# simeoncarstens/binf

Hardware: AMD Instinct MI355X
Metric: chain*leapfrog-steps/sec, 1024-d Gaussian (higher is better)
Workload: dtype f64

## Files before the change

binf_amd/csrc/hmc_gauss.hip:

```cpp
#include "hmc_gauss_kernel.hpp"

namespace binf {

template <int TMAX, bool REGULAR, int LW, bool UDT = false, int HC = -1, bool FS = false>
static hipError_t launch_n_trl(const GaussNArgs &a, bool unit, bool fma, dim3 grid,
                               hipStream_t st)
{
    constexpr int BS = (LW == 3) ? 512 : 256;
    constexpr int R = GAUSS_RNG_HBM;
    constexpr bool FU = FS && gauss_fastsum_built(TMAX, HC, true);
    constexpr bool FN = FS && gauss_fastsum_built(TMAX, HC, false);
    if (unit) {
        if (fma) hmc_gauss_persist_kernel<TMAX, REGULAR, true, true, LW, R, UDT, HC, FU><<<grid, BS, 0, st>>>(a);
        else     hmc_gauss_persist_kernel<TMAX, REGULAR, true, false, LW, R, UDT, HC, FU><<<grid, BS, 0, st>>>(a);
    } else {
        if (fma) hmc_gauss_persist_kernel<TMAX, REGULAR, false, true, LW, R, UDT, HC, FN><<<grid, BS, 0, st>>>(a);
        else     hmc_gauss_persist_kernel<TMAX, REGULAR, false, false, LW, R, UDT, HC, FN><<<grid, BS, 0, st>>>(a);
    }
    return hipGetLastError();
}

static bool gauss_uniform_dt(const GaussNArgs &a)
{
    return a.dt_chain == nullptr && a.n_adapt == 0;
}

template <int TMAX, int HC>
static hipError_t launch_n_th(const GaussNArgs &a, bool unit, bool fma, dim3 grid,
                              hipStream_t st)
{
    if constexpr (HC == 3) {
        if (a.e_before == nullptr && a.e_after == nullptr) {
            if constexpr (TMAX == 16) {
                if (unit && gauss_uniform_dt(a) && gauss_onesum_domain(a)) {
                    constexpr int R = GAUSS_RNG_HBM;
                    if (fma) hmc_gauss_persist_kernel<16, true, true, true, 0, R, true, 3, true, true><<<grid, 256, 0, st>>>(a);
                    else     hmc_gauss_persist_kernel<16, true, true, false, 0, R, true, 3, true, true><<<grid, 256, 0, st>>>(a);
                    return hipGetLastError();
                }
            }
            if (gauss_uniform_dt(a))
                return launch_n_trl<TMAX, true, 0, true, HC, true>(a, unit, fma, grid, st);
            return launch_n_trl<TMAX, true, 0, false, HC, true>(a, unit, fma, grid, st);
        }
    }
    if (gauss_uniform_dt(a))
        return launch_n_trl<TMAX, true, 0, true, HC>(a, unit, fma, grid, st);
    return launch_n_trl<TMAX, true, 0, false, HC>(a, unit, fma, grid, st);
}

template <int TMAX>
static hipError_t launch_n_t(const GaussNArgs &a, bool regular, bool unit, bool fma,
                             dim3 grid, hipStream_t st)
{
    if (!regular)
        return launch_n_trl<TMAX, false, 0>(a, unit, fma, grid, st);
    if (a.H == 0) return launch_n_th<TMAX, 0>(a, unit, fma, grid, st);
    if constexpr (TMAX >= 12) {
        if (a.H == 1) return launch_n_th<TMAX, 1>(a, unit, fma, grid, st);
        if (a.H == 2) return launch_n_th<TMAX, 2>(a, unit, fma, grid, st);
        if (a.H == 3) return launch_n_th<TMAX, 3>(a, unit, fma, grid, st);
    }
    return hipErrorNotSupported;
}

template <int LW>
static hipError_t launch_n_wide(const GaussNArgs &a, bool regular, bool unit, bool fma,
                                dim3 grid, hipStream_t st)
{
    return regular ? launch_n_trl<16, true, LW>(a, unit, fma, grid, st)
                   : launch_n_trl<16, false, LW>(a, unit, fma, grid, st);
}

}

using namespace binf;

extern "C" int32_t binf_hmc_sample_n_gauss_f64(
    const double *q0, const double *p0, const double *u, double *q_out,
    double *samples, uint8_t *accepted, int64_t *n_accepted, double *e_before,
    double *e_after, double timestep, double *dt_chain, int64_t C, int64_t D,
    int32_t nsteps, int32_t n, int32_t thin, double k, double x0,
    int32_t n_adapt, double uprate, double downrate, int32_t mode, void *stream)
{
    if (C < 0 || D < 1 || nsteps < 1 || n < 1 || thin < 1 || n_adapt < 0)
        return fail(BINF_E_ARG, "hmc_sample_gauss: need C>=0, D>=1, nsteps>=1, n>=1, thin>=1, n_adapt>=0");
    if (mode != BINF_MODE_EXACT && mode != BINF_MODE_FMA)
        return fail(BINF_E_ARG, "hmc_sample_gauss: unknown mode %d", mode);
    if (C == 0) return 0;
    if (!q0 || !p0 || !u || !q_out)
        return fail(BINF_E_ARG, "hmc_sample_gauss: null buffer");
    if (n_adapt > 0 && !dt_chain)
        return fail(BINF_E_ARG, "hmc_sample_gauss: adaption needs dt_chain");
    if (D > 8192)
        return fail(BINF_E_UNSUPPORTED, "hmc_sample_gauss: D=%lld > 8192 not covered by the fused kernel", (long long)D);
    const GaussPlan plan = gauss_plan(C, D);
    const int32_t H = plan.H;
    if (H > 6)
        return fail(BINF_E_UNSUPPORTED, "hmc_sample_gauss: pairwise tree height %d > 6 for D=%lld", H, (long long)D);
    const int LW = plan.LW;
    const int64_t bytes = C * D * (int64_t)sizeof(double);
    const char *qo = (const char *)q_out, *qi = (const char *)q0, *pi = (const char *)p0;
    if ((qo != qi && qo < qi + bytes && qi < qo + bytes) ||
        (qo < pi + bytes * n && pi < qo + bytes))
        return fail(BINF_E_ALIAS, "hmc_sample_gauss: q_out overlaps q0/p0 (only q_out == q0 is allowed)");

    const int tneed = plan.tneed;
    const bool regular = plan.regular;
    GaussNArgs a;
    a.q0 = q0; a.p0 = p0; a.u = u; a.q_out = q_out; a.samples = samples;
    a.accepted = accepted; a.n_accepted = n_accepted; a.e_before = e_before;
    a.e_after = e_after; a.dt_chain = dt_chain; a.timestep = timestep; a.k = k;
    a.x0 = x0; a.uprate = uprate; a.downrate = downrate; a.C = C;
    a.D = (int32_t)D; a.nsteps = nsteps; a.H = H; a.n = n; a.thin = thin;
    a.n_adapt = n_adapt < n ? n_adapt : n;
    a.rng_seed = 0; a.rng_offset = 0; a.chain_offset = 0; a.p_dump = nullptr; a.u_dump = nullptr;
    gauss_derived_args(a);

    const int64_t blocks = plan.blocks;
    if (blocks > 0x7fffffffLL)
        return fail(BINF_E_UNSUPPORTED, "hmc_sample_gauss: too many chains");
    dim3 grid((unsigned)blocks);
    hipStream_t st = (hipStream_t)stream;
    const bool unit = (k == 1.0 && x0 == 0.0);
    const bool fma = (mode == BINF_MODE_FMA);
    hipError_t e;
    const int split = (LW == 0) ? gauss_split_factor(C, H, regular, tneed) : 1;
    if (split > 1)        e = launch_gauss_split(a, tneed, split, unit, fma, st);
    else if (LW == 1)     e = launch_n_wide<1>(a, regular && tneed == 16, unit, fma, grid, st);
    else if (LW == 2)     e = launch_n_wide<2>(a, regular && tneed == 16, unit, fma, grid, st);
    else if (LW == 3)     e = launch_n_wide<3>(a, regular && tneed == 16, unit, fma, grid, st);
    else if (tneed <= 1)  e = launch_n_t<1>(a, regular && tneed == 1, unit, fma, grid, st);
    else if (tneed <= 2)  e = launch_n_t<2>(a, regular && tneed == 2, unit, fma, grid, st);
    else if (tneed <= 4)  e = launch_n_t<4>(a, regular && tneed == 4, unit, fma, grid, st);
    else if (tneed <= 8)  e = launch_n_t<8>(a, regular && tneed == 8, unit, fma, grid, st);
    else if (tneed <= 12) e = launch_n_t<12>(a, regular && tneed == 12, unit, fma, grid, st);
    else                  e = launch_n_t<16>(a, regular && tneed == 16, unit, fma, grid, st);
    if (e != hipSuccess) return hip_fail(e, "hmc_gauss_persist_kernel launch");
    return 0;
}

extern "C" int32_t binf_hmc_gauss_waves_per_chain(int64_t C, int64_t D)
{
    if (C < 1 || D < 1 || D > 8192) return 0;
    const GaussPlan p = gauss_plan(C, D);
    if (p.H > 6) return 0;
    if (p.LW > 0) return 1 << p.LW;
    return gauss_split_factor(C, p.H, p.regular, p.tneed);
}

extern "C" int32_t binf_hmc_sample_gauss_f64(
    const double *q0, const double *p0, const double *u, double *q_out,
    uint8_t *accepted, int64_t *n_accepted, double *e_before, double *e_after,
    double timestep, double *dt_chain, int64_t C, int64_t D, int32_t nsteps,
    double k, double x0, int32_t adapt, double uprate, double downrate,
    int32_t mode, void *stream)
{
    if (C > 0 && D >= 1 && nsteps >= 1 && q0 && p0 && u && q_out && !accepted)
        return fail(BINF_E_ARG, "hmc_sample_gauss: null buffer");
    return binf_hmc_sample_n_gauss_f64(q0, p0, u, q_out, nullptr, accepted,
                                       n_accepted, e_before, e_after, timestep,
                                       dt_chain, C, D, nsteps, 1, 1, k, x0,
                                       adapt ? 1 : 0, uprate, downrate, mode,
                                       stream);
}
```

binf_amd/csrc/hmc_gauss_kernel.hpp:

```cpp
#pragma once
#include "gauss_common.hpp"
#include "xoshiro.hpp"

namespace binf {

enum { GAUSS_RNG_HBM = 0, GAUSS_RNG_FUSED = 1, GAUSS_RNG_DUMP = 2 };

constexpr int gauss_wpb(int LW, int RNG) { return (LW == 3 || RNG != GAUSS_RNG_HBM) ? 8 : 4; }

constexpr int GAUSS_STEP_UNROLL = 4;
constexpr int gauss_step_unroll(int TMAX, bool REGULAR, bool UNIT, bool FMA, int LW, int RNG)
{
    if (!REGULAR || LW != 0 || !UNIT) return 1;
    if ((TMAX == 12 && !FMA) || (TMAX == 4 && RNG == GAUSS_RNG_FUSED)) return 1;
    return GAUSS_STEP_UNROLL;
}

constexpr int GAUSS_PRIO_WINDOW = 4;
constexpr bool gauss_wave_priority(int LW, int RNG, int HC)
{
    return LW == 0 && RNG == GAUSS_RNG_HBM && HC == 3;
}

__device__ __forceinline__ void gauss_set_priority(int prio)
{
    switch (prio & 3) {
    case 0: __builtin_amdgcn_s_setprio(0); break;
    case 1: __builtin_amdgcn_s_setprio(1); break;
    case 2: __builtin_amdgcn_s_setprio(2); break;
    default: __builtin_amdgcn_s_setprio(3); break;
    }
}

constexpr int GAUSS_REDO_GS = 2;
template <int TMAX, int GS, bool UNIT, bool FMA>
__device__ inline bool gauss_exact_accept(const GaussNArgs &a, const double *qs, const double (*qs_lds)[64],
                                          int lane, const double *pc, double dt, double hdt, double c_lp,
                                          double u)
{
    LaneSum s0 = {0.0, 0.0}, spb = {0.0, 0.0}, sqa = {0.0, 0.0}, spa = {0.0, 0.0};
#pragma unroll 1
    for (int g = 0; g < TMAX / GS; ++g) {
        double qq[GS], pp[GS];
#pragma unroll
        for (int i = 0; i < GS; ++i) {
            const int t = g * GS + i;
            qq[i] = qs_lds ? qs_lds[t][lane] : qs[8 * t];
            pp[i] = pc[8 * t];
        }
#pragma unroll
        for (int i = 0; i < GS; ++i) {
            const int t = g * GS + i;
            const double d = UNIT ? qq[i] : qq[i] - a.x0;
            lane_sum_add<true>(s0, d * d, t, TMAX);
            lane_sum_add<true>(spb, pp[i] * pp[i], t, TMAX);
        }
#pragma unroll
        for (int i = 0; i < GS; ++i)
            pp[i] = kick<FMA>(pp[i], hdt, gauss_grad<UNIT>(qq[i], a.k, a.x0));
#pragma unroll 1
        for (int l = 0; l < a.nsteps - 1; ++l) {
#pragma unroll
            for (int i = 0; i < GS; ++i) {
                qq[i] = drift<FMA>(qq[i], pp[i], dt);
                pp[i] = kick<FMA>(pp[i], dt, gauss_grad<UNIT>(qq[i], a.k, a.x0));
            }
        }
#pragma unroll
        for (int i = 0; i < GS; ++i) {
            const int t = g * GS + i;
            qq[i] = drift<FMA>(qq[i], pp[i], dt);
            pp[i] = kick<FMA>(pp[i], hdt, gauss_grad<UNIT>(qq[i], a.k, a.x0));
            const double d = UNIT ? qq[i] : qq[i] - a.x0;
            lane_sum_add<true>(sqa, d * d, t, TMAX);
            lane_sum_add<true>(spa, pp[i] * pp[i], t, TMAX);
        }
    }
    const double r = chain_sums_shared(sqa.r, spa.r, spb.r, s0.r, true);
    const double Eb = -(c_lp * lane_value_f64<12>(r)) + 0.5 * lane_value_f64<8>(r);
    const double Ea = -(c_lp * lane_value_f64<0>(r)) + 0.5 * lane_value_f64<4>(r);
    return metropolis_accept<true>(u, -(Ea - Eb));
}

constexpr bool gauss_fastsum_built(int TMAX, int HC, bool UNIT) { return HC == 3 && (TMAX == 16 || !UNIT); }

template <int TMAX, bool REGULAR, bool UNIT, bool FMA, int LW, int RNG = GAUSS_RNG_HBM, bool UDT = false,
          int HC = -1, bool FASTSUM = false, bool ONESUM = false>
__global__ void __launch_bounds__(64 * gauss_wpb(LW, RNG))
hmc_gauss_persist_kernel(const GaussNArgs a)
{
    static_assert(HC < 0 || (REGULAR && LW == 0), "compile-time tree height: regular one-wave chains only");
    constexpr bool FIXED = HC >= 0;
    constexpr int HF = FIXED ? HC : 0;
    constexpr bool SHARED = HC == 3;
    static_assert(!FASTSUM || (SHARED && RNG == GAUSS_RNG_HBM), "fused sums: the shared-tree kernels, draws from HBM");
    static_assert(!ONESUM || (FASTSUM && UNIT && UDT), "two sums: the unit Gaussian, one step size for the batch");
    constexpr bool EARLY = FIXED && UNIT && !SHARED;
    constexpr int WPB = gauss_wpb(LW, RNG);
    constexpr int WPC = 1 << LW;
    __shared__ double xch[WPB];
    __shared__ double ubc[WPB];
    constexpr int GS = (TMAX % 8 == 0) ? 8 : ((TMAX % 4 == 0) ? 4 : TMAX);
    constexpr int NG = TMAX / GS;
    constexpr int USTEP = gauss_step_unroll(TMAX, REGULAR, UNIT, FMA, LW, RNG);
    constexpr bool PRIO = gauss_wave_priority(LW, RNG, HC);
    __shared__ double stash[RNG == GAUSS_RNG_DUMP ? 1 : WPB][RNG == GAUSS_RNG_DUMP ? 1 : TMAX][64];
    __shared__ double zx[RNG == GAUSS_RNG_HBM ? 1 : XZIG_C + 1];
    if (RNG != GAUSS_RNG_HBM) {
        xzig_load_table(zx, threadIdx.x, WPB * 64);
        __syncthreads();
    }

    const int lane = threadIdx.x & 63;
    const int wib = threadIdx.x >> 6;
    const int64_t wave = (int64_t)blockIdx.x * WPB + wib;
    const int H = FIXED ? HC : a.H;
    const int lg = (LW > 0) ? 6 : 3 + H;
    const int slot = lane & ((1 << lg) - 1);
    const int j = slot & 7;
    const int wchain = wib & (WPC - 1);
    const int grp = (LW > 0) ? ((wchain << 3) | (lane >> 3)) : (slot >> 3);
    const bool writer = (LW > 0) ? (wchain == 0 && lane == 0) : (slot == 0);

    int off, n, leafdepth, canonical;
    if (REGULAR) {
        n = 8 * TMAX;
        off = grp * n;
        leafdepth = H;
        canonical = 1;
    } else {
        const Leaf L = pairwise_leaf(a.D, H, grp);
        off = L.off;
        n = L.len;
        leafdepth = L.depth;
        canonical = L.canonical;
    }
    const int T = (n >= 8) ? (n >> 3) : 0;
    const int rem = (n >= 8) ? (n & 7) : n;

    const int64_t raw = (LW > 0) ? (int64_t)blockIdx.x * (WPB / WPC) + (wib >> LW)
                                 : (wave << (6 - lg)) + (lane >> lg);
    const bool cvalid = raw < a.C;
    const int64_t chain = cvalid ? raw : a.C - 1;
    const int64_t CD = a.C * (int64_t)a.D;
    const int64_t base = chain * (int64_t)a.D + off + j;

    double dt = (UDT || !a.dt_chain) ? a.timestep : a.dt_chain[chain];
    double uu = 0.0;
    if (RNG == GAUSS_RNG_HBM) uu = a.u[chain];
    Xo128 gen = {0u, 0u, 0u, 0u};
    uint64_t gen_stream = 0;
    if (RNG != GAUSS_RNG_HBM) {
        const int cgrp = grp & ~((1 << (H - leafdepth)) - 1);
        gen_stream = (uint64_t)(chain + a.chain_offset) * (uint64_t)(8 << H) + (uint64_t)(cgrp * 8 + j);
    }
    __builtin_amdgcn_sched_barrier(0);

    double q[TMAX], pa[GS], pb[GS];
#pragma unroll
    for (int t = 0; t < GS; ++t) {
        const bool m = REGULAR || (8 * t + j < n);
        q[t] = (m && RNG != GAUSS_RNG_DUMP) ? a.q0[base + 8 * t] : 0.0;
    }
    if (RNG == GAUSS_RNG_HBM) {
#pragma unroll
        for (int i = 0; i < GS; ++i) {
            const bool m = REGULAR || (8 * i + j < n);
            pa[i] = m ? a.p0[base + 8 * i] : 0.0;
        }
    }
#pragma unroll
    for (int t = GS; t < TMAX; ++t) {
        const bool m = REGULAR || (8 * t + j < n);
        q[t] = (m && RNG != GAUSS_RNG_DUMP) ? a.q0[base + 8 * t] : 0.0;
    }

    const double c_lp = SHARED ? a.c_lp : -0.5 * a.k;
    LaneSum s0 = {0.0, 0.0};
    double Sq_state = 0.0;
    int64_t nacc = 0;

    const bool stash_lds = !(REGULAR && ((a.samples && a.thin == 1) || a.n == 1));
    double *rec = a.samples;
    const double *prev = a.q0;
    int rec_wait = a.thin;

    for (int s = 0; s < a.n; ++s) {
        if (PRIO) {
            const int left = (a.n - 1 - s) / GAUSS_PRIO_WINDOW;
            gauss_set_priority(left < 3 ? left : 3);
        }
        const double hdt = (UDT && SHARED) ? a.half_timestep : 0.5 * dt;
        if (RNG != GAUSS_RNG_HBM) gen = xo_seed(gen_stream, a.rng_seed, a.rng_offset + (uint64_t)s);
        if (RNG != GAUSS_RNG_DUMP && stash_lds) {
#pragma unroll
            for (int t = 0; t < TMAX; ++t) stash[wib][t][lane] = q[t];
        }

        const bool more = s + 1 < a.n;
        const double *pc = a.p0 + (int64_t)s * CD + base;
        const double *pn = more ? pc + CD : pc;
        double un = 0.0;
        if (RNG == GAUSS_RNG_HBM) un = a.u[(int64_t)(more ? s + 1 : s) * a.C + chain];

        LaneSum spb = {0.0, 0.0}, sqa = {0.0, 0.0}, spa = {0.0, 0.0};
        double Spb = 0.0;
#pragma unroll
        for (int g = 0; g < NG; ++g) {
            double(&cur)[GS] = (RNG == GAUSS_RNG_HBM && (g & 1)) ? pb : pa;
            double(&nxt)[GS] = (RNG == GAUSS_RNG_HBM && (g & 1)) ? pa : pb;
            if (RNG != GAUSS_RNG_HBM) {
                unsigned want = 0;
#pragma unroll
                for (int i = 0; i < GS; ++i)
                    if (REGULAR || (8 * (g * GS + i) + j < n)) want |= 1u << i;
                xzig_normals<GS>(cur, want, gen, zx);
                if (RNG == GAUSS_RNG_DUMP) {
                    if (cvalid && canonical) {
                        double *go = a.p_dump + (int64_t)s * CD + base;
#pragma unroll
                        for (int i = 0; i < GS; ++i)
                            if (want & (1u << i)) go[8 * (g * GS + i)] = cur[i];
                    }
                    continue;
                }
            } else if (g + 1 < NG) {
#pragma unroll
                for (int i = 0; i < GS; ++i) {
                    const int t = (g + 1) * GS + i;
                    const bool m = REGULAR || (8 * t + j < n);
                    nxt[i] = m ? pc[8 * t] : 0.0;
                }
            } else {
#pragma unroll
                for (int i = 0; i < GS; ++i) {
                    const bool m = REGULAR || (8 * i + j < n);
                    nxt[i] = m ? pn[8 * i] : 0.0;
                }
            }
            (void)nxt;
#pragma unroll
            for (int i = 0; i < GS; ++i)
                asm volatile("" : "+v"(cur[i]), "+v"(q[g * GS + i]));
            if (s == 0) {
#pragma unroll
                for (int i = 0; i < GS; ++i) {
                    const int t = g * GS + i;
                    const double d = UNIT ? q[t] : q[t] - a.x0;
                    if (FASTSUM) lane_sum_fused(s0, d, t);
                    else lane_sum_add<REGULAR>(s0, d * d, t, T);
                }
                if (FIXED && !SHARED && g == NG - 1) {
                    double v[1] = {s0.r};
                    chain_sum_finish_fixed<HF, 1>(v, lane);
                    Sq_state = v[0];
                }
            }
#pragma unroll
            for (int i = 0; i < GS; ++i) {
                if (FASTSUM) lane_sum_fused(spb, cur[i], g * GS + i);
                else lane_sum_add<REGULAR>(spb, cur[i] * cur[i], g * GS + i, T);
            }
            __builtin_amdgcn_sched_barrier(0);
            if (EARLY && g == NG - 1) {
                double v[1] = {spb.r};
                chain_sum_finish_fixed<HF, 1>(v, lane);
                Spb = v[0];
            }
#pragma unroll
            for (int i = 0; i < GS; ++i) {
                const int t = g * GS + i;
                cur[i] = kick<FMA>(cur[i], hdt, gauss_grad<UNIT>(q[t], a.k, a.x0));
            }
            if (EARLY && g == NG - 1) asm volatile("" : "+v"(Spb));
            if (USTEP == 1) {
                for (int l = 0; l < a.nsteps - 1; ++l) {
#pragma unroll
                    for (int i = 0; i < GS; ++i) {
                        const int t = g * GS + i;
                        q[t] = drift<FMA>(q[t], cur[i], dt);
                        cur[i] = kick<FMA>(cur[i], dt, gauss_grad<UNIT>(q[t], a.k, a.x0));
                    }
                }
            } else {
                const auto step = [&]() {
#pragma unroll
                    for (int i = 0; i < GS; ++i) {
                        const int t = g * GS + i;
                        q[t] = drift<FMA>(q[t], cur[i], dt);
                        cur[i] = kick<FMA>(cur[i], dt, gauss_grad<UNIT>(q[t], a.k, a.x0));
                    }
                };
                static_assert((USTEP & (USTEP - 1)) == 0, "the remainder below goes by the bits of its count");
                const int nl = a.nsteps > 1 ? a.nsteps - 1 : 0;
#pragma unroll 1
                for (int m = nl / USTEP; m > 0; --m) {
#pragma unroll
                    for (int k = 0; k < USTEP; ++k) step();
                }
#pragma unroll
                for (int b = USTEP >> 1; b > 0; b >>= 1) {
                    if (nl & b) {
#pragma unroll
                        for (int k = 0; k < b; ++k) step();
                    }
                }
            }
#pragma unroll
            for (int i = 0; i < GS; ++i) {
                const int t = g * GS + i;
                q[t] = drift<FMA>(q[t], cur[i], dt);
                if (!ONESUM) cur[i] = kick<FMA>(cur[i], hdt, gauss_grad<UNIT>(q[t], a.k, a.x0));
            }
#pragma unroll
            for (int i = 0; i < GS; ++i) {
                const int t = g * GS + i;
                const double d = UNIT ? q[t] : q[t] - a.x0;
                if (ONESUM) {
                    lane_sum_fused(sqa, d, t);
                } else if (FASTSUM) {
                    lane_sum_fused(sqa, d, t);
                    lane_sum_fused(spa, cur[i], t);
                } else {
                    lane_sum_add<REGULAR>(sqa, d * d, t, T);
                    lane_sum_add<REGULAR>(spa, cur[i] * cur[i], t, T);
                }
            }
            if (ONESUM)
                asm volatile("" : "+v"(sqa.r), "+v"(spb.r));
            else if (EARLY && g == NG - 1)
                asm volatile("" : "+v"(sqa.r), "+v"(spa.r));
            else
                asm volatile("" : "+v"(sqa.r), "+v"(spa.r), "+v"(spb.r));
            __builtin_amdgcn_sched_barrier(0);
        }
        if (RNG != GAUSS_RNG_HBM) {
            const double ud = xo_uniform53(gen);
            if (LW == 0) {
                uu = shfl_f64(ud, lane & ~((1 << lg) - 1));
            } else {
                if (wchain == 0 && lane == 0) ubc[wib] = ud;
                __syncthreads();
                uu = ubc[wib & ~(WPC - 1)];
                __syncthreads();
            }
            if (RNG == GAUSS_RNG_DUMP) {
                if (cvalid && writer) a.u_dump[(int64_t)s * a.C + chain] = uu;
                continue;
            }
        }
        if (RNG == GAUSS_RNG_HBM && (NG & 1)) {
#pragma unroll
            for (int i = 0; i < GS; ++i) pa[i] = pb[i];
        }
        double Sqa, Spa = 0.0;
        if (ONESUM) {
            const double r = chain_sums_shared2(sqa.r, spb.r, s0.r, s == 0);
            Sqa = lane_value_f64<0>(r);
            Spb = lane_value_f64<4>(r);
            if (s == 0) Sq_state = lane_value_f64<8>(r);
        } else if (SHARED) {
            const double r = chain_sums_shared(sqa.r, spa.r, spb.r, s0.r, s == 0);
            Sqa = lane_value_f64<0>(r);
            Spa = lane_value_f64<4>(r);
            Spb = lane_value_f64<8>(r);
            if (s == 0) Sq_state = lane_value_f64<12>(r);
        } else if (FIXED) {
            if (EARLY) {
                double v[2] = {sqa.r, spa.r};
                chain_sum_finish_fixed<HF, 2>(v, lane);
                Sqa = v[0];
                Spa = v[1];
            } else {
                double v[3] = {spb.r, sqa.r, spa.r};
                chain_sum_finish_fixed<HF, 3>(v, lane);
                Spb = v[0];
                Sqa = v[1];
                Spa = v[2];
            }
        } else {
            if (s == 0)
                Sq_state = chain_sum_finish<REGULAR, LW>(s0, T, rem, lane, H, leafdepth, xch, wib);
            Spb = chain_sum_finish<REGULAR, LW>(spb, T, rem, lane, H, leafdepth, xch, wib);
            Sqa = chain_sum_finish<REGULAR, LW>(sqa, T, rem, lane, H, leafdepth, xch, wib);
            Spa = chain_sum_finish<REGULAR, LW>(spa, T, rem, lane, H, leafdepth, xch, wib);
        }
        const double Eb = -(c_lp * Sq_state) + 0.5 * Spb;
        const double Ea = -(c_lp * Sqa) + 0.5 * Spa;

        bool acc;
        if (FASTSUM) {
            const double xt = ONESUM ? -(a.c_dh * (Sqa - Sq_state)) : -(Ea - Eb);
            const double delta = ONESUM ? a.f_dh * ((Eb + Eb) + __builtin_fabs(xt)) : 0x1p-46 * (Eb + Ea);
            const int dec = accept_decide(uu, xt, delta);
            acc = dec == GAUSS_ACCEPT;
            if (__builtin_amdgcn_ballot_w64(dec == GAUSS_UNDECIDED || !(c_lp < 0.0)) != 0) {
                acc = gauss_exact_accept<TMAX, GAUSS_REDO_GS, UNIT, FMA>(
                    a, prev + base, stash_lds ? stash[wib] : nullptr, lane, pc, dt, hdt, c_lp, uu);
                __builtin_amdgcn_s_waitcnt(0);
            }
        } else {
            acc = metropolis_accept<SHARED>(uu, -(Ea - Eb));
        }

        if (!UDT && s < a.n_adapt)
            dt = acc ? dt * a.uprate : dt * a.downrate;
        if (cvalid && writer) {
            const int64_t o = (int64_t)s * a.C + chain;
            if (a.accepted) a.accepted[o] = acc ? 1 : 0;
            if (!ONESUM) {
                if (a.e_before) a.e_before[o] = Eb;
                if (a.e_after) a.e_after[o] = Ea;
            }
        }
        if (acc) {
            Sq_state = Sqa;
            nacc += 1;
        } else {
            if (stash_lds) {
#pragma unroll
                for (int t = 0; t < TMAX; ++t) q[t] = stash[wib][t][lane];
            } else {
#pragma unroll
                for (int t = 0; t < TMAX; ++t) q[t] = prev[base + 8 * t];
            }
            __builtin_amdgcn_s_waitcnt(0);
        }
        if (a.samples && --rec_wait == 0) {
            rec_wait = a.thin;
            if (cvalid && canonical) {
                double *go = rec + base;
#pragma unroll
                for (int t = 0; t < TMAX; ++t)
                    if (REGULAR || (8 * t + j < n)) go[8 * t] = q[t];
            }
            prev = rec;
            rec += CD;
        }
        if (RNG == GAUSS_RNG_HBM) uu = un;
    }
    if (RNG == GAUSS_RNG_DUMP) return;
    if (PRIO) __builtin_amdgcn_s_setprio(0);

    if (cvalid && writer) {
        if (a.n_accepted) a.n_accepted[chain] += nacc;
        if (!UDT && a.n_adapt > 0 && a.dt_chain) a.dt_chain[chain] = dt;
    }
    if (cvalid && canonical) {
        double *go = a.q_out + base;
#pragma unroll
        for (int t = 0; t < TMAX; ++t)
            if (REGULAR || (8 * t + j < n)) go[8 * t] = q[t];
    }
}


}
```

Measured before the change: 5.577 billion.

## Use 16-byte paired loads/stores for one-wave 1024-d Gaussian HMC chains

After: 5.658 billion, median of 6. 1.5% higher.

```diff
diff --git a/binf_amd/csrc/hmc_gauss.hip b/binf_amd/csrc/hmc_gauss.hip
--- a/binf_amd/csrc/hmc_gauss.hip
+++ b/binf_amd/csrc/hmc_gauss.hip
@@ -25,6 +25,12 @@
     return a.dt_chain == nullptr && a.n_adapt == 0;
 }
 
+static bool gauss_wide_aligned(const GaussNArgs &a)
+{
+    const uintptr_t any = (uintptr_t)a.q0 | (uintptr_t)a.p0 | (uintptr_t)a.samples | (uintptr_t)a.q_out;
+    return (any & 15) == 0;
+}
+
 template <int TMAX, int HC>
 static hipError_t launch_n_th(const GaussNArgs &a, bool unit, bool fma, dim3 grid,
                               hipStream_t st)
@@ -34,6 +40,10 @@
             if constexpr (TMAX == 16) {
                 if (unit && gauss_uniform_dt(a) && gauss_onesum_domain(a)) {
                     constexpr int R = GAUSS_RNG_HBM;
+                    if (!fma && gauss_wide_aligned(a)) {
+                        hmc_gauss_persist_kernel<16, true, true, false, 0, R, true, 3, true, true, true><<<grid, 256, 0, st>>>(a);
+                        return hipGetLastError();
+                    }
                     if (fma) hmc_gauss_persist_kernel<16, true, true, true, 0, R, true, 3, true, true><<<grid, 256, 0, st>>>(a);
                     else     hmc_gauss_persist_kernel<16, true, true, false, 0, R, true, 3, true, true><<<grid, 256, 0, st>>>(a);
                     return hipGetLastError();
diff --git a/binf_amd/csrc/hmc_gauss_kernel.hpp b/binf_amd/csrc/hmc_gauss_kernel.hpp
--- a/binf_amd/csrc/hmc_gauss_kernel.hpp
+++ b/binf_amd/csrc/hmc_gauss_kernel.hpp
@@ -33,19 +33,21 @@
 }
 
 constexpr int GAUSS_REDO_GS = 2;
-template <int TMAX, int GS, bool UNIT, bool FMA>
+template <int TMAX, int GS, bool UNIT, bool FMA, bool WIDE = false>
 __device__ inline bool gauss_exact_accept(const GaussNArgs &a, const double *qs, const double (*qs_lds)[64],
                                           int lane, const double *pc, double dt, double hdt, double c_lp,
                                           double u)
 {
     LaneSum s0 = {0.0, 0.0}, spb = {0.0, 0.0}, sqa = {0.0, 0.0}, spa = {0.0, 0.0};
+    const int e0 = 128 * (lane >> 3) + (lane & 7);
 #pragma unroll 1
     for (int g = 0; g < TMAX / GS; ++g) {
         double qq[GS], pp[GS];
 #pragma unroll
         for (int i = 0; i < GS; ++i) {
             const int t = g * GS + i;
-            qq[i] = qs_lds ? qs_lds[t][lane] : qs[8 * t];
+            if (WIDE) qq[i] = qs_lds ? (&qs_lds[0][0])[e0 + 8 * t] : qs[8 * t];
+            else qq[i] = qs_lds ? qs_lds[t][lane] : qs[8 * t];
             pp[i] = pc[8 * t];
         }
 #pragma unroll
@@ -84,11 +86,26 @@
 
 constexpr bool gauss_fastsum_built(int TMAX, int HC, bool UNIT) { return HC == 3 && (TMAX == 16 || !UNIT); }
 
+typedef double gauss_d2 __attribute__((ext_vector_type(2)));
+__device__ __forceinline__ void gauss_ld2(double &x, double &y, const double *p)
+{
+    const gauss_d2 v = *reinterpret_cast<const gauss_d2 *>(p);
+    x = v.x;
+    y = v.y;
+}
+__device__ __forceinline__ void gauss_st2(double *p, double x, double y)
+{
+    const gauss_d2 v = {x, y};
+    *reinterpret_cast<gauss_d2 *>(p) = v;
+}
+
 template <int TMAX, bool REGULAR, bool UNIT, bool FMA, int LW, int RNG = GAUSS_RNG_HBM, bool UDT = false,
-          int HC = -1, bool FASTSUM = false, bool ONESUM = false>
+          int HC = -1, bool FASTSUM = false, bool ONESUM = false, bool WIDE = false>
 __global__ void __launch_bounds__(64 * gauss_wpb(LW, RNG))
 hmc_gauss_persist_kernel(const GaussNArgs a)
 {
+    static_assert(!WIDE || (ONESUM && TMAX == 16 && HC == 3 && REGULAR && LW == 0),
+                  "16-byte ownership: the two-sum kernel of one 1024-element chain per wave");
     static_assert(HC < 0 || (REGULAR && LW == 0), "compile-time tree height: regular one-wave chains only");
     constexpr bool FIXED = HC >= 0;
     constexpr int HF = FIXED ? HC : 0;
@@ -104,7 +121,7 @@
     constexpr int NG = TMAX / GS;
     constexpr int USTEP = gauss_step_unroll(TMAX, REGULAR, UNIT, FMA, LW, RNG);
     constexpr bool PRIO = gauss_wave_priority(LW, RNG, HC);
-    __shared__ double stash[RNG == GAUSS_RNG_DUMP ? 1 : WPB][RNG == GAUSS_RNG_DUMP ? 1 : TMAX][64];
+    alignas(WIDE ? 16 : 8) __shared__ double stash[RNG == GAUSS_RNG_DUMP ? 1 : WPB][RNG == GAUSS_RNG_DUMP ? 1 : TMAX][64];
     __shared__ double zx[RNG == GAUSS_RNG_HBM ? 1 : XZIG_C + 1];
     if (RNG != GAUSS_RNG_HBM) {
         xzig_load_table(zx, threadIdx.x, WPB * 64);
@@ -143,7 +160,9 @@
     const bool cvalid = raw < a.C;
     const int64_t chain = cvalid ? raw : a.C - 1;
     const int64_t CD = a.C * (int64_t)a.D;
-    const int64_t base = chain * (int64_t)a.D + off + j;
+    const int64_t base_np = chain * (int64_t)a.D + off + j;
+    constexpr int WR0 = TMAX / 4;
+    const int64_t base = WIDE ? chain * (int64_t)a.D + 2 * lane + 128 * WR0 : base_np;
 
     double dt = (UDT || !a.dt_chain) ? a.timestep : a.dt_chain[chain];
     double uu = 0.0;
@@ -157,22 +176,31 @@
     __builtin_amdgcn_sched_barrier(0);
 
     double q[TMAX], pa[GS], pb[GS];
-#pragma unroll
-    for (int t = 0; t < GS; ++t) {
-        const bool m = REGULAR || (8 * t + j < n);
-        q[t] = (m && RNG != GAUSS_RNG_DUMP) ? a.q0[base + 8 * t] : 0.0;
-    }
-    if (RNG == GAUSS_RNG_HBM) {
-#pragma unroll
-        for (int i = 0; i < GS; ++i) {
-            const bool m = REGULAR || (8 * i + j < n);
-            pa[i] = m ? a.p0[base + 8 * i] : 0.0;
-        }
-    }
-#pragma unroll
-    for (int t = GS; t < TMAX; ++t) {
-        const bool m = REGULAR || (8 * t + j < n);
-        q[t] = (m && RNG != GAUSS_RNG_DUMP) ? a.q0[base + 8 * t] : 0.0;
+    if constexpr (WIDE) {
+#pragma unroll
+        for (int r = 0; r < GS / 2; ++r) gauss_ld2(q[2 * r], q[2 * r + 1], a.q0 + base + 128 * (r - WR0));
+#pragma unroll
+        for (int r = 0; r < GS / 2; ++r) gauss_ld2(pa[2 * r], pa[2 * r + 1], a.p0 + base + 128 * (r - WR0));
+#pragma unroll
+        for (int r = GS / 2; r < TMAX / 2; ++r) gauss_ld2(q[2 * r], q[2 * r + 1], a.q0 + base + 128 * (r - WR0));
+    } else {
+#pragma unroll
+        for (int t = 0; t < GS; ++t) {
+            const bool m = REGULAR || (8 * t + j < n);
+            q[t] = (m && RNG != GAUSS_RNG_DUMP) ? a.q0[base + 8 * t] : 0.0;
+        }
+        if (RNG == GAUSS_RNG_HBM) {
+#pragma unroll
+            for (int i = 0; i < GS; ++i) {
+                const bool m = REGULAR || (8 * i + j < n);
+                pa[i] = m ? a.p0[base + 8 * i] : 0.0;
+            }
+        }
+#pragma unroll
+        for (int t = GS; t < TMAX; ++t) {
+            const bool m = REGULAR || (8 * t + j < n);
+            q[t] = (m && RNG != GAUSS_RNG_DUMP) ? a.q0[base + 8 * t] : 0.0;
+        }
     }
 
     const double c_lp = SHARED ? a.c_lp : -0.5 * a.k;
@@ -193,8 +221,14 @@
         const double hdt = (UDT && SHARED) ? a.half_timestep : 0.5 * dt;
         if (RNG != GAUSS_RNG_HBM) gen = xo_seed(gen_stream, a.rng_seed, a.rng_offset + (uint64_t)s);
         if (RNG != GAUSS_RNG_DUMP && stash_lds) {
-#pragma unroll
-            for (int t = 0; t < TMAX; ++t) stash[wib][t][lane] = q[t];
+            if constexpr (WIDE) {
+#pragma unroll
+                for (int r = 0; r < TMAX / 2; ++r)
+                    gauss_st2(&stash[wib][0][0] + 128 * r + 2 * lane, q[2 * r], q[2 * r + 1]);
+            } else {
+#pragma unroll
+                for (int t = 0; t < TMAX; ++t) stash[wib][t][lane] = q[t];
+            }
         }
 
         const bool more = s + 1 < a.n;
@@ -224,6 +258,10 @@
                     }
                     continue;
                 }
+            } else if (WIDE) {
+                const double *pg = (g + 1 < NG) ? pc + 128 * ((g + 1) * (GS / 2)) : pn;
+#pragma unroll
+                for (int r = 0; r < GS / 2; ++r) gauss_ld2(nxt[2 * r], nxt[2 * r + 1], pg + 128 * (r - WR0));
             } else if (g + 1 < NG) {
 #pragma unroll
                 for (int i = 0; i < GS; ++i) {
@@ -395,8 +433,9 @@
             const int dec = accept_decide(uu, xt, delta);
             acc = dec == GAUSS_ACCEPT;
             if (__builtin_amdgcn_ballot_w64(dec == GAUSS_UNDECIDED || !(c_lp < 0.0)) != 0) {
-                acc = gauss_exact_accept<TMAX, GAUSS_REDO_GS, UNIT, FMA>(
-                    a, prev + base, stash_lds ? stash[wib] : nullptr, lane, pc, dt, hdt, c_lp, uu);
+                acc = gauss_exact_accept<TMAX, GAUSS_REDO_GS, UNIT, FMA, WIDE>(
+                    a, prev + base_np, stash_lds ? stash[wib] : nullptr, lane, pc + (base_np - base), dt, hdt,
+                    c_lp, uu);
                 __builtin_amdgcn_s_waitcnt(0);
             }
         } else {
@@ -417,7 +456,14 @@
             Sq_state = Sqa;
             nacc += 1;
         } else {
-            if (stash_lds) {
+            if (WIDE && stash_lds) {
+#pragma unroll
+                for (int r = 0; r < TMAX / 2; ++r)
+                    gauss_ld2(q[2 * r], q[2 * r + 1], &stash[wib][0][0] + 128 * r + 2 * lane);
+            } else if (WIDE) {
+#pragma unroll
+                for (int r = 0; r < TMAX / 2; ++r) gauss_ld2(q[2 * r], q[2 * r + 1], prev + base + 128 * (r - WR0));
+            } else if (stash_lds) {
 #pragma unroll
                 for (int t = 0; t < TMAX; ++t) q[t] = stash[wib][t][lane];
             } else {
@@ -430,9 +476,14 @@
             rec_wait = a.thin;
             if (cvalid && canonical) {
                 double *go = rec + base;
-#pragma unroll
-                for (int t = 0; t < TMAX; ++t)
-                    if (REGULAR || (8 * t + j < n)) go[8 * t] = q[t];
+                if constexpr (WIDE) {
+#pragma unroll
+                    for (int r = 0; r < TMAX / 2; ++r) gauss_st2(go + 128 * (r - WR0), q[2 * r], q[2 * r + 1]);
+                } else {
+#pragma unroll
+                    for (int t = 0; t < TMAX; ++t)
+                        if (REGULAR || (8 * t + j < n)) go[8 * t] = q[t];
+                }
             }
             prev = rec;
             rec += CD;
@@ -448,11 +499,16 @@
     }
     if (cvalid && canonical) {
         double *go = a.q_out + base;
-#pragma unroll
-        for (int t = 0; t < TMAX; ++t)
-            if (REGULAR || (8 * t + j < n)) go[8 * t] = q[t];
-    }
-}
-
-
-}
+        if constexpr (WIDE) {
+#pragma unroll
+            for (int r = 0; r < TMAX / 2; ++r) gauss_st2(go + 128 * (r - WR0), q[2 * r], q[2 * r + 1]);
+        } else {
+#pragma unroll
+            for (int t = 0; t < TMAX; ++t)
+                if (REGULAR || (8 * t + j < n)) go[8 * t] = q[t];
+        }
+    }
+}
+
+
+}
```
